# dspcraft/dsc

Measured on AMD Instinct MI355X. Metric: batched 1-D rfft GSamples/s, higher is better.
Workload: dtype f32

## Files before the change

dsc_amd/csrc/fft_r2c_64k.hip:

```cpp
#include "kernels.h"

#include <hip/hip_runtime.h>

#include <cmath>
#include <cstdlib>
#include <utility>

namespace {

typedef float f2 __attribute__((ext_vector_type(2)));

struct cf { float x, y; };
__device__ __forceinline__ cf operator+(cf a, cf b) { return cf{a.x + b.x, a.y + b.y}; }
__device__ __forceinline__ cf operator-(cf a, cf b) { return cf{a.x - b.x, a.y - b.y}; }
__device__ __forceinline__ cf to_cf(f2 a) { return cf{a.x, a.y}; }
__device__ __forceinline__ f2 to_f2(cf a) { return f2{a.x, a.y}; }

constexpr int kM = 32768;
constexpr int kRowPitch = 34;
constexpr int kPlaneFloats = 1024 * kRowPitch;
constexpr int kLdsBytes = kPlaneFloats * 4 + 1024 * 8;
constexpr int kTabEntries = 1024;

constexpr int kAuxW1024 = 0, kAuxW32768 = 1024, kAuxW65536 = 2048, kAuxEntries = 3072;

__host__ __device__ constexpr int br5(int x) {
    return ((x & 1) << 4) | ((x & 2) << 2) | (x & 4) | ((x & 8) >> 2) | ((x & 16) >> 4);
}

__device__ constexpr float kCos64[17] = {
    1.0f, 0.99518472667219688624f, 0.98078528040323044913f, 0.95694033573220886494f,
    0.92387953251128675613f, 0.88192126434835502971f, 0.83146961230254523708f, 0.77301045336273696081f,
    0.70710678118654752440f, 0.63439328416364549822f, 0.55557023301960222474f, 0.47139673682599764856f,
    0.38268343236508977173f, 0.29028467725446236764f, 0.19509032201612826785f, 0.09801714032956060199f,
    0.0f};

__device__ constexpr float root64_re(int q) {
    q &= 63;
    return q <= 16 ? kCos64[q] : q <= 32 ? -kCos64[32 - q] : q <= 48 ? -kCos64[q - 32] : kCos64[64 - q];
}
__device__ constexpr float root64_im(int q) {
    q &= 63;
    return q <= 16 ? -kCos64[16 - q] : q <= 32 ? -kCos64[q - 16] : q <= 48 ? kCos64[48 - q] : kCos64[q - 48];
}

__device__ __forceinline__ cf cmul(cf a, cf w) {
    return cf{a.x * w.x - a.y * w.y, a.x * w.y + a.y * w.x};
}
__device__ __forceinline__ cf cmul_conj(cf a, cf w) {
    return cf{a.x * w.x + a.y * w.y, a.y * w.x - a.x * w.y};
}

template<bool INV, int M, int K>
__device__ __forceinline__ cf mul_root(cf d) {
    constexpr float c8 = 0.70710678118654752440f;
    if constexpr (K == 0) {
        return d;
    } else if constexpr (4 * K == M) {
        return INV ? cf{-d.y, d.x} : cf{d.y, -d.x};
    } else if constexpr (8 * K == M) {
        return INV ? cf{(d.x - d.y) * c8, (d.x + d.y) * c8} : cf{(d.x + d.y) * c8, (d.y - d.x) * c8};
    } else if constexpr (8 * K == 3 * M) {
        return INV ? cf{-(d.x + d.y) * c8, (d.x - d.y) * c8} : cf{(d.y - d.x) * c8, -(d.x + d.y) * c8};
    } else {
        constexpr float wr = root64_re(K * (64 / M));
        constexpr float wi = INV ? -root64_im(K * (64 / M)) : root64_im(K * (64 / M));
        return cf{d.x * wr - d.y * wi, d.x * wi + d.y * wr};
    }
}

#ifdef DSC_DFT32_DIF
template<bool INV, int M, int G, int... K>
__device__ __forceinline__ void dif_group(cf (&v)[32], std::integer_sequence<int, K...>) {
    (([&] {
         const cf u = v[G + K] + v[G + K + M / 2];
         const cf d = v[G + K] - v[G + K + M / 2];
         v[G + K] = u;
         v[G + K + M / 2] = mul_root<INV, M, K>(d);
     }()),
     ...);
}

template<bool INV, int M, int... G>
__device__ __forceinline__ void dif_stage(cf (&v)[32], std::integer_sequence<int, G...>) {
    (dif_group<INV, M, G * M>(v, std::make_integer_sequence<int, M / 2>{}), ...);
}

template<bool INV>
__device__ __forceinline__ void dft32(cf (&v)[32]) {
    dif_stage<INV, 32>(v, std::make_integer_sequence<int, 1>{});
    dif_stage<INV, 16>(v, std::make_integer_sequence<int, 2>{});
    dif_stage<INV, 8>(v, std::make_integer_sequence<int, 4>{});
    dif_stage<INV, 4>(v, std::make_integer_sequence<int, 8>{});
    dif_stage<INV, 2>(v, std::make_integer_sequence<int, 16>{});
}


#else
constexpr double kCos64d[17] = {
    1.0, 0.99518472667219688624, 0.98078528040323044913, 0.95694033573220886494,
    0.92387953251128675613, 0.88192126434835502971, 0.83146961230254523708, 0.77301045336273696081,
    0.70710678118654752440, 0.63439328416364549822, 0.55557023301960222474, 0.47139673682599764856,
    0.38268343236508977173, 0.29028467725446236764, 0.19509032201612826785, 0.09801714032956060199,
    0.0};

template<bool INV, int E>
__device__ __forceinline__ void dit_butterfly(cf &a, cf &b) {
    if constexpr (E == 0) {
        const cf u = a + b, d = a - b;
        a = u; b = d;
    } else if constexpr (E == 8) {
        const cf u = INV ? cf{a.x - b.y, a.y + b.x} : cf{a.x + b.y, a.y - b.x};
        const cf d = INV ? cf{a.x + b.y, a.y - b.x} : cf{a.x - b.y, a.y + b.x};
        a = u; b = d;
    } else {
        constexpr double c = E <= 8 ? kCos64d[2 * E] : -kCos64d[32 - 2 * E];
        constexpr double sn = (E <= 8 ? kCos64d[16 - 2 * E] : kCos64d[2 * E - 16]);
        constexpr double s = INV ? sn : -sn;
        if constexpr ((c < 0 ? -c : c) >= sn) {
            constexpr float t = (float) (s / c), cc = (float) c;
            float p, q;
            if constexpr (t == 1.0f) { p = b.x - b.y; q = b.y + b.x; }
            else if constexpr (t == -1.0f) { p = b.x + b.y; q = b.y - b.x; }
            else { p = __builtin_fmaf(-t, b.y, b.x); q = __builtin_fmaf(t, b.x, b.y); }
            const cf u = cf{__builtin_fmaf(cc, p, a.x), __builtin_fmaf(cc, q, a.y)};
            const cf d = cf{__builtin_fmaf(-cc, p, a.x), __builtin_fmaf(-cc, q, a.y)};
            a = u; b = d;
        } else {
            constexpr float r = (float) (c / s), ss = (float) s;
            const float pn = __builtin_fmaf(-r, b.x, b.y);
            const float q = __builtin_fmaf(r, b.y, b.x);
            const cf u = cf{__builtin_fmaf(-ss, pn, a.x), __builtin_fmaf(ss, q, a.y)};
            const cf d = cf{__builtin_fmaf(ss, pn, a.x), __builtin_fmaf(-ss, q, a.y)};
            a = u; b = d;
        }
    }
}

constexpr int brev_bits(int x, int bits) {
    int r = 0;
    for (int i = 0; i < bits; ++i) r |= ((x >> i) & 1) << (bits - 1 - i);
    return r;
}

template<bool INV, int S, int G, int... J>
__device__ __forceinline__ void dit_group(cf (&v)[32], std::integer_sequence<int, J...>) {
    constexpr int H = 32 >> S;
    constexpr int E = brev_bits(G, S - 1) * (16 >> (S - 1));
    (dit_butterfly<INV, E>(v[2 * H * G + J], v[2 * H * G + J + H]), ...);
}

template<bool INV, int S, int... G>
__device__ __forceinline__ void dit_stage(cf (&v)[32], std::integer_sequence<int, G...>) {
    (dit_group<INV, S, G>(v, std::make_integer_sequence<int, (32 >> S)>{}), ...);
}

template<bool INV>
__device__ __forceinline__ void dft32(cf (&v)[32]) {
    dit_stage<INV, 1>(v, std::make_integer_sequence<int, 1>{});
    dit_stage<INV, 2>(v, std::make_integer_sequence<int, 2>{});
    dit_stage<INV, 3>(v, std::make_integer_sequence<int, 4>{});
    dit_stage<INV, 4>(v, std::make_integer_sequence<int, 8>{});
    dit_stage<INV, 5>(v, std::make_integer_sequence<int, 16>{});
}
#endif

typedef unsigned int u2 __attribute__((ext_vector_type(2)));
typedef unsigned int u4 __attribute__((ext_vector_type(4)));
typedef float f4 __attribute__((ext_vector_type(4)));

template<int COMP>
__device__ __forceinline__ void plane_write(float *plane, int wbase, const cf (&v)[32]) {
    float *lo16 = plane + wbase;
    float *hi16 = lo16 + 16 * (32 * kRowPitch);
#pragma unroll
    for (int p = 0; p < 32; ++p) {
        const int slot = br5(p);
        const float val = COMP == 0 ? v[p].x : v[p].y;
        if (slot < 16) lo16[slot * (32 * kRowPitch)] = val;
        else           hi16[(slot - 16) * (32 * kRowPitch)] = val;
    }
}
template<int COMP>
__device__ __forceinline__ void plane_read(const float *plane, int row, cf (&v)[32]) {
    const f2 *r = (const f2 *) (plane + row * kRowPitch);
#pragma unroll
    for (int m = 0; m < 16; ++m) {
        const f2 t = r[m];
        if (COMP == 0) { v[2 * m].x = t.x; v[2 * m + 1].x = t.y; }
        else           { v[2 * m].y = t.x; v[2 * m + 1].y = t.y; }
    }
}

__device__ __forceinline__ void lds_barrier() {
    __builtin_amdgcn_fence(__ATOMIC_RELEASE, "workgroup", "local");
    __builtin_amdgcn_s_barrier();
    __builtin_amdgcn_fence(__ATOMIC_ACQUIRE, "workgroup", "local");
}

__device__ __forceinline__ float bperm(int byte_addr, float x) {
    return __int_as_float(__builtin_amdgcn_ds_bpermute(byte_addr, __float_as_int(x)));
}

__device__ __forceinline__ int column_of(int wave, int lane) {
    int kp = lane < 32 ? 32 * wave + lane : 1024 - 32 * wave - (63 - lane);
    return kp == 1024 ? 512 : kp;
}

#ifdef DSC_R2C64K_PROBE
#define PROBE_ARGS , int io_on
#define PROBE_NULL , 1
#define IO_ON io_on
#else
#define PROBE_ARGS
#define PROBE_NULL
#define IO_ON 1
#endif

__device__ __forceinline__ int thread_id(int wave_sgpr) {
    int zero;
    asm volatile("v_mov_b32 %0, 0" : "=v"(zero));
    const int lane = __builtin_amdgcn_mbcnt_hi(-1, __builtin_amdgcn_mbcnt_lo(-1, zero));
    return (wave_sgpr << 6) | lane;
}

#ifndef DSC_STREAM_AUX
#define DSC_STREAM_AUX 2
#endif
constexpr int kStream = DSC_STREAM_AUX;
__device__ __forceinline__ cf load_c(__amdgpu_buffer_rsrc_t r, int voff, int soff) {
    return to_cf(__builtin_bit_cast(f2, __builtin_amdgcn_raw_buffer_load_b64(r, voff, soff, kStream)));
}
#ifndef DSC_FILTER_EARLY_LOADS
#define DSC_FILTER_EARLY_LOADS 4
#endif
#ifndef DSC_IRFFT_PIN_PASS3
#define DSC_IRFFT_PIN_PASS3 1
#endif
#ifndef DSC_IRFFT_EARLY_PAIRS
#define DSC_IRFFT_EARLY_PAIRS 4
#endif
#ifndef DSC_IRFFT_LOAD_AUX
#define DSC_IRFFT_LOAD_AUX 0
#endif
__device__ __forceinline__ cf load_c_spec(__amdgpu_buffer_rsrc_t r, int voff, int soff) {
    return to_cf(__builtin_bit_cast(f2, __builtin_amdgcn_raw_buffer_load_b64(r, voff, soff, DSC_IRFFT_LOAD_AUX)));
}
__device__ __forceinline__ cf load_c_cached(__amdgpu_buffer_rsrc_t r, int voff, int soff) {
    return to_cf(__builtin_bit_cast(f2, __builtin_amdgcn_raw_buffer_load_b64(r, voff, soff, 0)));
}
template<int POLICY>
__device__ __forceinline__ void store_c(cf a, __amdgpu_buffer_rsrc_t r, int voff, int soff) {
    __builtin_amdgcn_raw_buffer_store_b64(__builtin_bit_cast(u2, to_f2(a)), r, voff, soff, POLICY);
}

__device__ __forceinline__ void exchange(float *plane, int wbase, int row, const cf (&src)[32], cf (&dst)[32]) {
    plane_write<0>(plane, wbase, src);
    lds_barrier();
    plane_read<0>(plane, row, dst);
    lds_barrier();
    plane_write<1>(plane, wbase, src);
    lds_barrier();
    plane_read<1>(plane, row, dst);
    lds_barrier();
}

struct no_hook { __device__ __forceinline__ void operator()() const {} };

template<bool INV, typename Hook = no_hook>
__device__ __forceinline__ void three_passes(cf (&v)[32], float *plane, const f2 *w1024, const f2 *aux, int wave_sgpr,
                                             bool mirrored_in, bool mirrored_out, Hook before_pass3 = Hook{}) {
    dft32<INV>(v);
    cf u[32];
    {
        const int t = thread_id(wave_sgpr);
        const int col = mirrored_in ? column_of(t >> 6, t & 63) : t;
        const int hi = col >> 5;
#pragma unroll
        for (int r1 = 1; r1 < 32; ++r1) {
            const cf w = to_cf(w1024[hi * r1]);
            v[br5(r1)] = INV ? cmul_conj(v[br5(r1)], w) : cmul(v[br5(r1)], w);
        }
        exchange(plane, (col & 31) * kRowPitch + hi, t, v, u);
    }
    dft32<INV>(u);
    {
        const int t = thread_id(wave_sgpr);
        const int hi = t >> 5, lo = t & 31;
        const cf tw2_base = to_cf(aux[kAuxW32768 + hi * lo]);
        u[0] = INV ? cmul_conj(u[0], tw2_base) : cmul(u[0], tw2_base);
#pragma unroll
        for (int r2 = 1; r2 < 32; ++r2) {
            const cf w = cmul(tw2_base, to_cf(w1024[lo * r2]));
            u[br5(r2)] = INV ? cmul_conj(u[br5(r2)], w) : cmul(u[br5(r2)], w);
        }
        const int col_out = mirrored_out ? column_of(t >> 6, t & 63) : t;
        exchange(plane, hi * kRowPitch + lo, col_out, u, v);
    }
    before_pass3();
    dft32<INV>(v);
}

__device__ __forceinline__ void real_pair(cf p, cf q, cf wq, float hs, cf &out_k, cf &out_mk) {
    const cf s = cf{p.x + q.x, p.y - q.y};
    const cf d = cf{p.x - q.x, p.y + q.y};
    const cf wd = cmul(d, wq);
    out_k = cf{hs * s.x + wd.x, hs * s.y + wd.y};
    out_mk = cf{hs * s.x - wd.x, wd.y - hs * s.y};
}

__device__ __forceinline__ int partner_byte_addr(int wave, int lane) {
    return ((wave == 0 && (lane == 63 || lane == 0)) ? lane : 63 - lane) * 4;
}

#ifndef DSC_R2C64K_HELPERS_ONLY
__global__ __launch_bounds__(1024) void rfft64k_kernel(const float *__restrict__ x, f2 *__restrict__ X, int batch,
                                                       const f2 *__restrict__ aux, int in_pitch, int in_len PROBE_ARGS) {
    extern __shared__ __attribute__((aligned(16))) float lds[];
    float *plane = lds;
    f2 *w1024 = (f2 *) (lds + kPlaneFloats);
    w1024[threadIdx.x] = aux[kAuxW1024 + threadIdx.x];
    __syncthreads();

    const int wave_sgpr = __builtin_amdgcn_readfirstlane(threadIdx.x >> 6);

    cf v[32];
    {
        const int row0 = blockIdx.x;
        const __amdgpu_buffer_rsrc_t r0 = __builtin_amdgcn_make_buffer_rsrc(
            (void *) (x + (size_t) row0 * in_pitch), 0, row0 < batch ? in_len * 4 * IO_ON : 0, 0x00020000);
        const int load_off = thread_id(wave_sgpr) * 8;
#pragma unroll
        for (int j1 = 0; j1 < 32; ++j1) v[j1] = load_c(r0, load_off, j1 * 8192);
    }

    for (int row = blockIdx.x; row < batch; row += gridDim.x) {
        const int next_row = row + gridDim.x;
        const __amdgpu_buffer_rsrc_t rnext = __builtin_amdgcn_make_buffer_rsrc(
            (void *) (x + (size_t) next_row * in_pitch), 0, next_row < batch ? in_len * 4 * IO_ON : 0, 0x00020000);
        const __amdgpu_buffer_rsrc_t rout =
            __builtin_amdgcn_make_buffer_rsrc((void *) (X + (size_t) row * (kM + 1)), 0, (kM + 1) * 8 * IO_ON, 0x00020000);

        three_passes<false>(v, plane, w1024, aux, wave_sgpr, false, true);

        const int t4 = thread_id(wave_sgpr);
        const int lane = t4 & 63, wave = t4 >> 6;
        const int kp = column_of(wave, lane);
        const int partner_addr = partner_byte_addr(wave, lane);
        cf xk[16], xm[16];
        const cf zmid = v[br5(16)];
        if (wave_sgpr == 0) {
#pragma unroll
            for (int r = 16; r < 31; ++r) v[br5(r)] = lane == 0 ? v[br5(r + 1)] : v[br5(r)];
            v[br5(31)] = lane == 0 ? v[br5(0)] : v[br5(31)];
        }
#pragma unroll
        for (int k3 = 0; k3 < 16; ++k3) {
            const int src = 31 - br5(k3);
            xm[k3].x = bperm(partner_addr, v[src].x);
            xm[k3].y = bperm(partner_addr, v[src].y);
        }
        {
            const cf wpost = to_cf(aux[kAuxW65536 + kp]);
            const cf post_base = cf{0.5f * wpost.y, -0.5f * wpost.x};
#pragma unroll
            for (int k3 = 0; k3 < 16; ++k3) {
                const cf c = cf{root64_re(k3), root64_im(k3)};
                const cf w = k3 == 0 ? post_base : cmul(post_base, c);
                real_pair(v[br5(k3)], xm[k3], w, 0.5f, xk[k3], xm[k3]);
            }
        }

        f2 *stage = (f2 *) plane;
        const int skew = (int) ((((size_t) (X + (size_t) row * (kM + 1))) >> 3) & 15);
#pragma unroll
        for (int k3 = 0; k3 < 16; ++k3) stage[kp + 1024 * k3] = to_f2(xk[k3]);
        const cf xk15 = xk[15];
        const int load_off = thread_id(wave_sgpr) * 8;
#pragma unroll
        for (int j1 = 0; j1 < 16; ++j1) v[j1] = load_c(rnext, load_off, j1 * 8192);
        lds_barrier();
#pragma unroll
        for (int m = 0; m < 8; ++m) {
            const int k = 2 * (t4 + 1024 * m) - skew;
            if (m > 0 || k >= 0) {
                const f2 lo2 = stage[k], hi2 = stage[k + 1];
                const f4 q = f4{lo2.x, lo2.y, hi2.x, hi2.y};
                __builtin_amdgcn_raw_buffer_store_b128(__builtin_bit_cast(u4, q), rout, k * 8, 0, kStream);
            } else if (m == 0 && k == -1) {
                __builtin_amdgcn_raw_buffer_store_b64(__builtin_bit_cast(u2, stage[0]), rout, 0, 0, kStream);
            }
            if (m & 1) __builtin_amdgcn_sched_barrier(0);
        }
        lds_barrier();
        constexpr int kStage2 = kM / 2 - 16;
#pragma unroll
        for (int k3 = 0; k3 < 16; ++k3) stage[(kM - kStage2) - kp - 1024 * k3] = to_f2(xm[k3]);
        if (kp >= 1009) stage[kp + 15 * 1024 - kStage2] = to_f2(xk15);
        if (t4 == 0) stage[kM / 2 - kStage2] = f2{zmid.x, -zmid.y};
#pragma unroll
        for (int j1 = 16; j1 < 32; ++j1) v[j1] = load_c(rnext, load_off, j1 * 8192);
        lds_barrier();
#pragma unroll
        for (int m = 0; m < 9; ++m) {
            if (m == 8 && wave != 0) break;
            const int k = kM / 2 + 2 * (t4 + 1024 * m) - skew;
            if (m < 8 || k + 1 <= kM) {
                const f2 lo2 = stage[k - kStage2], hi2 = stage[k + 1 - kStage2];
                const f4 q = f4{lo2.x, lo2.y, hi2.x, hi2.y};
                __builtin_amdgcn_raw_buffer_store_b128(__builtin_bit_cast(u4, q), rout, k * 8, 0, kStream);
            } else if (m == 8 && k == kM) {
                __builtin_amdgcn_raw_buffer_store_b64(__builtin_bit_cast(u2, stage[k - kStage2]), rout, k * 8, 0, kStream);
            }
            if (m & 1) __builtin_amdgcn_sched_barrier(0);
        }
        lds_barrier();
    }
}

#endif

__device__ __forceinline__ void inverse_prepass_direct(cf (&v)[32], cf y_mid, const f2 *aux, int wave_sgpr) {
    constexpr float kScale = 1.0f / (float) kM;
    const int t1 = thread_id(wave_sgpr);
    const int lane = t1 & 63, wave = t1 >> 6;
    const int c = column_of(wave, lane);
    const int partner_addr = partner_byte_addr(wave, lane);
    if (wave == 0 && lane == 0) { v[0].y = 0.f; v[16].y = 0.f; }
    const cf wpre = to_cf(aux[kAuxW65536 + c]);
    const cf wq_base = cf{0.5f * kScale * wpre.y, 0.5f * kScale * wpre.x};
#pragma unroll
    for (int half = 0; half < 2; ++half) {
        cf zm[8];
#pragma unroll
        for (int i = 0; i < 8; ++i) {
            const int a = half * 8 + i;
            const cf cj = cf{root64_re(a), -root64_im(a)};
            const cf wq = a == 0 ? wq_base : cmul(wq_base, cj);
            real_pair(v[a], v[16 + a], wq, 0.5f * kScale, v[a], zm[i]);
        }
#pragma unroll
        for (int i = 0; i < 8; ++i) {
            const int a = half * 8 + i;
            v[16 + a].x = bperm(partner_addr, zm[i].x);
            v[16 + a].y = bperm(partner_addr, zm[i].y);
        }
    }
    cf w[32];
#pragma unroll
    for (int r = 0; r < 16; ++r) { w[r] = v[r]; w[16 + r] = v[31 - r]; }
    if (wave == 0) {
#pragma unroll
        for (int r = 31; r > 16; --r) w[r] = lane == 0 ? w[r - 1] : w[r];
        w[16] = lane == 0 ? cf{kScale * y_mid.x, -kScale * y_mid.y} : w[16];
    }
#pragma unroll
    for (int r = 0; r < 32; ++r) v[r] = w[r];
}

template<typename IssueNext>
__device__ __forceinline__ void staged_time_store(cf (&v)[32], float *plane, __amdgpu_buffer_rsrc_t rout, int wave_sgpr,
                                                  IssueNext issue_next) {
    f2 *stage = (f2 *) plane;
    const int t4 = thread_id(wave_sgpr);
#pragma unroll
    for (int p = 0; p < 32; p += 2) stage[t4 + 1024 * br5(p)] = to_f2(v[p]);
    issue_next(true);
    lds_barrier();
#pragma unroll
    for (int m = 0; m < 8; ++m) {
        const int k = 2 * (t4 + 1024 * m);
        const f2 lo2 = stage[k], hi2 = stage[k + 1];
        const f4 q = f4{lo2.x, lo2.y, hi2.x, hi2.y};
        __builtin_amdgcn_raw_buffer_store_b128(__builtin_bit_cast(u4, q), rout, k * 8, 0, kStream);
        if (m & 1) __builtin_amdgcn_sched_barrier(0);
    }
    lds_barrier();
#pragma unroll
    for (int p = 1; p < 32; p += 2) stage[t4 + 1024 * (br5(p) - 16)] = to_f2(v[p]);
    issue_next(false);
    lds_barrier();
#pragma unroll
    for (int m = 0; m < 8; ++m) {
        const int k = 2 * (t4 + 1024 * m);
        const f2 lo2 = stage[k], hi2 = stage[k + 1];
        const f4 q = f4{lo2.x, lo2.y, hi2.x, hi2.y};
        __builtin_amdgcn_raw_buffer_store_b128(__builtin_bit_cast(u4, q), rout, (kM / 2 + k) * 8, 0, kStream);
        if (m & 1) __builtin_amdgcn_sched_barrier(0);
    }
    lds_barrier();
}

__device__ __forceinline__ void unzip_rows(cf (&v)[32]) {
    cf nxt[32];
#pragma unroll
    for (int a = 0; a < 16; ++a) { nxt[a] = v[2 * a]; nxt[16 + a] = v[2 * a + 1]; }
#pragma unroll
    for (int a = 0; a < 32; ++a) v[a] = nxt[a];
}

#ifndef DSC_R2C64K_HELPERS_ONLY
__global__ __launch_bounds__(1024) void irfft64k_kernel(const f2 *__restrict__ X, float *__restrict__ x, int batch,
                                                        const f2 *__restrict__ aux, int in_pitch, int in_len PROBE_ARGS) {
    extern __shared__ __attribute__((aligned(16))) float lds[];
    float *plane = lds;
    f2 *w1024 = (f2 *) (lds + kPlaneFloats);
    w1024[threadIdx.x] = aux[kAuxW1024 + threadIdx.x];
    __syncthreads();

    const int wave_sgpr = __builtin_amdgcn_readfirstlane(threadIdx.x >> 6);

    cf v[32];
    cf y_mid = cf{0.f, 0.f};
    {
        const int row0 = blockIdx.x;
        const __amdgpu_buffer_rsrc_t r0 = __builtin_amdgcn_make_buffer_rsrc(
            (void *) (X + (size_t) row0 * in_pitch), 0, row0 < batch ? in_len * 8 * IO_ON : 0, 0x00020000);
        const int t0 = thread_id(wave_sgpr);
        const int c = column_of(t0 >> 6, t0 & 63);
        const int pv = (kM - c - 15 * 1024) * 8;
#pragma unroll
        for (int a = 0; a < 16; ++a) {
            v[a] = load_c_spec(r0, c * 8, a * 8192);
            v[16 + a] = load_c_spec(r0, pv, (15 - a) * 8192);
        }
        if (c == 0) y_mid = load_c_spec(r0, (kM / 2) * 8, 0);
    }

    for (int row = blockIdx.x; row < batch; row += gridDim.x) {
        const int next_row = row + gridDim.x;
        const __amdgpu_buffer_rsrc_t rnext = __builtin_amdgcn_make_buffer_rsrc(
            (void *) (X + (size_t) next_row * in_pitch), 0, next_row < batch ? in_len * 8 * IO_ON : 0, 0x00020000);
        const __amdgpu_buffer_rsrc_t rout =
            __builtin_amdgcn_make_buffer_rsrc((void *) (x + (size_t) row * 65536), 0, 65536 * 4 * IO_ON, 0x00020000);

        inverse_prepass_direct(v, y_mid, aux, wave_sgpr);
        constexpr int kEarly = DSC_IRFFT_EARLY_PAIRS;
        cf early[kEarly > 0 ? 2 * kEarly : 1];
        three_passes<true>(v, plane, w1024, aux, wave_sgpr, true, false, [&]() {
            if constexpr (kEarly > 0) {
                const int t3 = thread_id(wave_sgpr);
                const int c3 = column_of(t3 >> 6, t3 & 63);
                const int pv3 = (kM - c3 - 15 * 1024) * 8;
#pragma unroll
                for (int a = 0; a < kEarly; ++a) {
                    early[2 * a] = load_c_spec(rnext, c3 * 8, a * 8192);
                    early[2 * a + 1] = load_c_spec(rnext, pv3, (15 - a) * 8192);
                }
            }
        });

#if DSC_IRFFT_PIN_PASS3
#pragma unroll
        for (int p = 0; p < 32; p += 8)
            asm volatile("" : "+v"(v[p].x), "+v"(v[p].y), "+v"(v[p + 1].x), "+v"(v[p + 1].y), "+v"(v[p + 2].x), "+v"(v[p + 2].y), "+v"(v[p + 3].x),
                         "+v"(v[p + 3].y), "+v"(v[p + 4].x), "+v"(v[p + 4].y), "+v"(v[p + 5].x), "+v"(v[p + 5].y), "+v"(v[p + 6].x), "+v"(v[p + 6].y),
                         "+v"(v[p + 7].x), "+v"(v[p + 7].y));
#endif
        const int t4 = thread_id(wave_sgpr);
        const int c = column_of(t4 >> 6, t4 & 63);
        const int pv = (kM - c - 15 * 1024) * 8;
        staged_time_store(v, plane, rout, wave_sgpr, [&](bool first_half) {
            if (first_half) {
                y_mid = cf{0.f, 0.f};
                if (c == 0) y_mid = load_c_spec(rnext, (kM / 2) * 8, 0);
#pragma unroll
                for (int i = 0; i < 8; ++i) {
                    v[2 * i] = load_c_spec(rnext, c * 8, (kEarly + i) * 8192);
                    v[16 + 2 * i] = load_c_spec(rnext, pv, (15 - kEarly - i) * 8192);
                }
            } else {
#pragma unroll
                for (int i = 0; i < 8 - kEarly; ++i) {
                    v[2 * i + 1] = load_c_spec(rnext, c * 8, (kEarly + 8 + i) * 8192);
                    v[17 + 2 * i] = load_c_spec(rnext, pv, (7 - kEarly - i) * 8192);
                }
            }
        });
        {
            cf nxt[32];
#pragma unroll
            for (int a = 0; a < 16; ++a) {
                if (a < kEarly)          { nxt[a] = early[2 * a];             nxt[16 + a] = early[2 * a + 1]; }
                else if (a < kEarly + 8) { nxt[a] = v[2 * (a - kEarly)];      nxt[16 + a] = v[16 + 2 * (a - kEarly)]; }
                else                     { nxt[a] = v[2 * (a - kEarly - 8) + 1]; nxt[16 + a] = v[17 + 2 * (a - kEarly - 8)]; }
            }
#pragma unroll
            for (int a = 0; a < 32; ++a) v[a] = nxt[a];
        }
    }
}

__global__ __launch_bounds__(1024) void filter64k_kernel(const float *__restrict__ x, const f2 *__restrict__ H,
                                                         float *__restrict__ y, int batch, const f2 *__restrict__ aux, int in_pitch,
                                                         int in_len) {
    extern __shared__ __attribute__((aligned(16))) float lds[];
    float *plane = lds;
    f2 *w1024 = (f2 *) (lds + kPlaneFloats);
    w1024[threadIdx.x] = aux[kAuxW1024 + threadIdx.x];
    __syncthreads();

    const int wave_sgpr = __builtin_amdgcn_readfirstlane(threadIdx.x >> 6);
    const __amdgpu_buffer_rsrc_t rh = __builtin_amdgcn_make_buffer_rsrc((void *) H, 0, (kM + 1) * 8, 0x00020000);
    constexpr float kScale = 1.0f / (float) kM;

    cf v[32];
    {
        const int row0 = blockIdx.x;
        const __amdgpu_buffer_rsrc_t r0 = __builtin_amdgcn_make_buffer_rsrc(
            (void *) (x + (size_t) row0 * in_pitch), 0, row0 < batch ? in_len * 4 : 0, 0x00020000);
        const int load_off = thread_id(wave_sgpr) * 8;
#pragma unroll
        for (int j1 = 0; j1 < 32; ++j1) v[j1] = load_c(r0, load_off, j1 * 8192);
    }
    for (int row = blockIdx.x; row < batch; row += gridDim.x) {
        const int next_row = row + gridDim.x;
        const __amdgpu_buffer_rsrc_t rnext = __builtin_amdgcn_make_buffer_rsrc(
            (void *) (x + (size_t) next_row * in_pitch), 0, next_row < batch ? in_len * 4 : 0, 0x00020000);
        const __amdgpu_buffer_rsrc_t rout =
            __builtin_amdgcn_make_buffer_rsrc((void *) (y + (size_t) row * 65536), 0, 65536 * 4, 0x00020000);
        three_passes<false>(v, plane, w1024, aux, wave_sgpr, false, true);

        {
            const int t1 = thread_id(wave_sgpr);
            const int lane = t1 & 63, wave = t1 >> 6;
            const int c = column_of(wave, lane);
            const int partner_addr = partner_byte_addr(wave, lane);
            const cf wc = to_cf(aux[kAuxW65536 + c]);
            const cf post_base = cf{0.5f * wc.y, -0.5f * wc.x};
            const cf pre_base = cf{0.5f * kScale * wc.y, 0.5f * kScale * wc.x};
            if (wave == 0) {
                const cf zmid = v[br5(16)];
                const cf hmid = load_c_cached(rh, (kM / 2) * 8, 0);
                const cf pmid = cmul(cf{zmid.x, -zmid.y}, hmid);
                v[br5(16)] = lane == 0 ? cf{kScale * pmid.x, -kScale * pmid.y} : v[br5(16)];
            }
            cf park = v[br5(16)];
            if (wave == 0) {
#pragma unroll
                for (int r = 16; r < 31; ++r) v[br5(r)] = lane == 0 ? v[br5(r + 1)] : v[br5(r)];
                v[br5(31)] = lane == 0 ? v[br5(0)] : v[br5(31)];
            }
#pragma unroll
            for (int part = 0; part < 8; ++part) {
                cf q[2], zm[2];
#pragma unroll
                for (int i = 0; i < 2; ++i) {
                    const int a = part * 2 + i;
                    q[i].x = bperm(partner_addr, v[br5(31 - a)].x);
                    q[i].y = bperm(partner_addr, v[br5(31 - a)].y);
                }
#pragma unroll
                for (int i = 0; i < 2; ++i) {
                    const int a = part * 2 + i;
                    const cf w64 = cf{root64_re(a), root64_im(a)};
                    cf xk, xm;
                    real_pair(v[br5(a)], q[i], a == 0 ? post_base : cmul(post_base, w64), 0.5f, xk, xm);
                    const cf hk = load_c_cached(rh, c * 8, a * 8192);
                    const cf hm = load_c_cached(rh, (kM - 15 * 1024 - c) * 8, (15 - a) * 8192);
                    cf pk = cmul(xk, hk), pm = cmul(xm, hm);
                    if (a == 0) {
                        pk.y = (c == 0) ? 0.f : pk.y;
                        pm.y = (c == 0) ? 0.f : pm.y;
                    }
                    const cf w64c = cf{root64_re(a), -root64_im(a)};
                    real_pair(pk, pm, a == 0 ? pre_base : cmul(pre_base, w64c), 0.5f * kScale, v[br5(a)], zm[i]);
                }
#pragma unroll
                for (int i = 0; i < 2; ++i) {
                    const int a = part * 2 + i;
                    v[br5(31 - a)].x = bperm(partner_addr, zm[i].x);
                    v[br5(31 - a)].y = bperm(partner_addr, zm[i].y);
                }
                __builtin_amdgcn_sched_barrier(0);
            }
            if (wave == 0) {
#pragma unroll
                for (int r = 31; r > 16; --r) v[br5(r)] = lane == 0 ? v[br5(r - 1)] : v[br5(r)];
                v[br5(16)] = lane == 0 ? park : v[br5(16)];
            }
        }
        cf z[32];
#pragma unroll
        for (int r = 0; r < 32; ++r) z[r] = v[br5(r)];
        constexpr int kEarlyX = DSC_FILTER_EARLY_LOADS;
        cf early[kEarlyX > 0 ? kEarlyX : 1];
        three_passes<true>(z, plane, w1024, aux, wave_sgpr, true, false, [&]() {
            if constexpr (kEarlyX > 0) {
                const int off = thread_id(wave_sgpr) * 8;
#pragma unroll
                for (int j1 = 0; j1 < kEarlyX; ++j1) early[j1] = load_c(rnext, off, j1 * 8192);
            }
        });
        {
            const int load_off = thread_id(wave_sgpr) * 8;
            staged_time_store(z, plane, rout, wave_sgpr, [&](bool first_half) {
                if (first_half) {
#pragma unroll
                    for (int i = 0; i < 16; ++i) z[2 * i] = load_c(rnext, load_off, (kEarlyX + i) * 8192);
                } else {
#pragma unroll
                    for (int i = 0; i < 16 - kEarlyX; ++i) z[2 * i + 1] = load_c(rnext, load_off, (kEarlyX + 16 + i) * 8192);
                }
            });
#pragma unroll
            for (int j1 = 0; j1 < 32; ++j1) v[j1] = j1 < kEarlyX ? early[j1] : j1 < kEarlyX + 16 ? z[2 * (j1 - kEarlyX)] : z[2 * (j1 - kEarlyX - 16) + 1];
        }
    }
}

#endif

}

#ifndef DSC_R2C64K_HELPERS_ONLY
size_t dsc_r2c64k_table_bytes() { return (size_t) kAuxEntries * sizeof(float) * 2; }

void dsc_r2c64k_build_tables(void *host_dst) {
    float *o = (float *) host_dst;
    auto put = [&](int at, long long k, long long n) {
        const long double a = -2.0L * 3.14159265358979323846264338327950288L * (long double) k / (long double) n;
        o[2 * at] = (float) cosl(a);
        o[2 * at + 1] = (float) sinl(a);
    };
    for (int m = 0; m < kTabEntries; ++m) {
        put(kAuxW1024 + m, m, 1024);
        put(kAuxW32768 + m, m, 32768);
        put(kAuxW65536 + m, m, 65536);
    }
    o[2 * (kAuxW1024 + 256)] = 0.f;  o[2 * (kAuxW1024 + 256) + 1] = -1.f;
    o[2 * (kAuxW1024 + 512)] = -1.f; o[2 * (kAuxW1024 + 512) + 1] = 0.f;
    o[2 * (kAuxW1024 + 768)] = 0.f;  o[2 * (kAuxW1024 + 768) + 1] = 1.f;
}

void dsc_launch_rfft64k(const float *x, void *X, int batch, int in_pitch, int in_len, const void *aux, int n_cu, hipStream_t stream) {
    if (batch <= 0) return;
    static unsigned long long attr_devices = 0;
    if (dsc_first_use_on_device(attr_devices)) {
        DSC_KERNEL_CHECK(hipFuncSetAttribute((const void *) rfft64k_kernel, hipFuncAttributeMaxDynamicSharedMemorySize, kLdsBytes));
    }
    const int grid = batch < n_cu ? batch : n_cu;
    DSC_LAUNCH(rfft64k_kernel, dim3(grid), dim3(1024), kLdsBytes, stream, x, (f2 *) X, batch, (const f2 *) aux, in_pitch, in_len PROBE_NULL);
}

void dsc_launch_irfft64k(const void *X, float *x, int batch, int in_pitch, int in_len, const void *aux, int n_cu, hipStream_t stream) {
    if (batch <= 0) return;
    static unsigned long long attr_devices = 0;
    if (dsc_first_use_on_device(attr_devices)) {
        DSC_KERNEL_CHECK(hipFuncSetAttribute((const void *) irfft64k_kernel, hipFuncAttributeMaxDynamicSharedMemorySize, kLdsBytes));
    }
    const int grid = batch < n_cu ? batch : n_cu;
    DSC_LAUNCH(irfft64k_kernel, dim3(grid), dim3(1024), kLdsBytes, stream, (const f2 *) X, x, batch, (const f2 *) aux, in_pitch, in_len PROBE_NULL);
}
void dsc_launch_filter64k(const float *s, const void *H, float *y, int batch, int in_pitch, int in_len, const void *aux, int n_cu,
                          hipStream_t stream) {
    if (batch <= 0) return;
    static unsigned long long attr_devices = 0;
    if (dsc_first_use_on_device(attr_devices)) {
        DSC_KERNEL_CHECK(hipFuncSetAttribute((const void *) filter64k_kernel, hipFuncAttributeMaxDynamicSharedMemorySize, kLdsBytes));
    }
    const int grid = batch < n_cu ? batch : n_cu;
    DSC_LAUNCH(filter64k_kernel, dim3(grid), dim3(1024), kLdsBytes, stream, s, (const f2 *) H, y, batch, (const f2 *) aux, in_pitch, in_len);
}
#endif
```

dsc_amd/csrc/fft_c2c_32k.hip:

```cpp
#define DSC_R2C64K_HELPERS_ONLY 1
#include "fft_r2c_64k.hip"

namespace {

template<bool INV, bool CAST>
__global__ __launch_bounds__(1024) void c2c32k_kernel(const f2 *__restrict__ z, f2 *__restrict__ Z, int batch, const f2 *__restrict__ aux,
                                                      int in_pitch, int in_len) {
    constexpr int EB = CAST ? 4 : 8;
    auto sample = [](__amdgpu_buffer_rsrc_t r, int voff, int soff) {
        if constexpr (CAST) return cf{__builtin_bit_cast(float, __builtin_amdgcn_raw_buffer_load_b32(r, voff, soff, kStream)), 0.0f};
        else return load_c(r, voff, soff);
    };
    extern __shared__ __attribute__((aligned(16))) float lds[];
    float *plane = lds;
    f2 *w1024 = (f2 *) (lds + kPlaneFloats);
    w1024[threadIdx.x] = aux[kAuxW1024 + threadIdx.x];
    __syncthreads();
    const int wave_sgpr = __builtin_amdgcn_readfirstlane(threadIdx.x >> 6);
    constexpr float kScale = 1.0f / (float) kM;

    cf v[32];
    {
        const int row0 = blockIdx.x;
        const __amdgpu_buffer_rsrc_t r0 = __builtin_amdgcn_make_buffer_rsrc(
            (void *) ((const char *) z + (size_t) row0 * in_pitch * EB), 0, row0 < batch ? in_len * EB : 0, 0x00020000);
        const int load_off = thread_id(wave_sgpr) * EB;
#pragma unroll
        for (int a = 0; a < 32; ++a) v[a] = sample(r0, load_off, a * 1024 * EB);
    }
    for (int row = blockIdx.x; row < batch; row += gridDim.x) {
        const int next_row = row + gridDim.x;
        const __amdgpu_buffer_rsrc_t rnext = __builtin_amdgcn_make_buffer_rsrc(
            (void *) ((const char *) z + (size_t) next_row * in_pitch * EB), 0, next_row < batch ? in_len * EB : 0, 0x00020000);
        const __amdgpu_buffer_rsrc_t rout = __builtin_amdgcn_make_buffer_rsrc((void *) (Z + (size_t) row * kM), 0, kM * 8, 0x00020000);
        three_passes<INV>(v, plane, w1024, aux, wave_sgpr, false, false);
        if (INV) {
#pragma unroll
            for (int p = 0; p < 32; ++p) v[p] = cf{v[p].x * kScale, v[p].y * kScale};
        }
        const int load_off = thread_id(wave_sgpr) * EB;
        staged_time_store(v, plane, rout, wave_sgpr, [&](bool first_half) {
            if (first_half) {
#pragma unroll
                for (int a = 0; a < 16; ++a) v[2 * a] = sample(rnext, load_off, a * 1024 * EB);
            } else {
#pragma unroll
                for (int a = 16; a < 32; ++a) v[2 * (a - 16) + 1] = sample(rnext, load_off, a * 1024 * EB);
            }
        });
        unzip_rows(v);
    }
}

}

void dsc_launch_fft32k_c32(const void *z, void *Z, int batch, int in_pitch, int in_len, bool inverse, bool cast, const void *aux, int n_cu,
                           hipStream_t stream) {
    if (batch <= 0) return;
    static unsigned long long attr_devices = 0;
    if (dsc_first_use_on_device(attr_devices)) {
        DSC_KERNEL_CHECK(hipFuncSetAttribute((const void *) c2c32k_kernel<false, false>, hipFuncAttributeMaxDynamicSharedMemorySize, kLdsBytes));
        DSC_KERNEL_CHECK(hipFuncSetAttribute((const void *) c2c32k_kernel<true, false>, hipFuncAttributeMaxDynamicSharedMemorySize, kLdsBytes));
        DSC_KERNEL_CHECK(hipFuncSetAttribute((const void *) c2c32k_kernel<false, true>, hipFuncAttributeMaxDynamicSharedMemorySize, kLdsBytes));
        DSC_KERNEL_CHECK(hipFuncSetAttribute((const void *) c2c32k_kernel<true, true>, hipFuncAttributeMaxDynamicSharedMemorySize, kLdsBytes));
    }
    const int grid = batch < n_cu ? batch : n_cu;
#define C2C32K(INV, CAST) DSC_LAUNCH((c2c32k_kernel<INV, CAST>), dim3(grid), dim3(1024), kLdsBytes, stream, (const f2 *) z, (f2 *) Z, batch, (const f2 *) aux, in_pitch, in_len)
    if (inverse) { if (cast) C2C32K(true, true); else C2C32K(true, false); }
    else         { if (cast) C2C32K(false, true); else C2C32K(false, false); }
#undef C2C32K
}
```

Measured before the change: 639.3.

## Relayout twiddle table and LDS staging for constant-offset reads and aligned stores

The W1024 table is rebuilt as a 32x32 product table indexed by (a,b), so each twiddle fetch becomes a base address plus an immediate offset, with no per-element multiply. Plane reads are forced into sixteen back-to-back ds_read_b64 instructions in inline asm, and plane writes are split into two loops over the even and odd output slots. The output staging buffer is pre-shifted by the skew so each store reads a single aligned f4 from LDS instead of two f2 loads. The inline asm with a full lgkmcnt wait and memory clobber limits how the compiler can schedule around it, and the changed table layout has to stay consistent with any other users of w1024 (e.g. the inverse path).

```diff
diff --git a/dsc_amd/csrc/fft_r2c_64k.hip b/dsc_amd/csrc/fft_r2c_64k.hip
--- a/dsc_amd/csrc/fft_r2c_64k.hip
+++ b/dsc_amd/csrc/fft_r2c_64k.hip
@@ -172,23 +172,45 @@
 template<int COMP>
 __device__ __forceinline__ void plane_write(float *plane, int wbase, const cf (&v)[32]) {
     float *lo16 = plane + wbase;
-    float *hi16 = lo16 + 16 * (32 * kRowPitch);
-#pragma unroll
-    for (int p = 0; p < 32; ++p) {
-        const int slot = br5(p);
-        const float val = COMP == 0 ? v[p].x : v[p].y;
-        if (slot < 16) lo16[slot * (32 * kRowPitch)] = val;
-        else           hi16[(slot - 16) * (32 * kRowPitch)] = val;
-    }
+    int wbase_hi = wbase + 16 * (32 * kRowPitch);
+    asm volatile("" : "+v"(wbase_hi));
+    float *hi16 = plane + wbase_hi;
+#pragma unroll
+    for (int p = 0; p < 32; p += 2) lo16[br5(p) * (32 * kRowPitch)] = COMP == 0 ? v[p].x : v[p].y;
+#pragma unroll
+    for (int p = 1; p < 32; p += 2) hi16[(br5(p) - 16) * (32 * kRowPitch)] = COMP == 0 ? v[p].x : v[p].y;
 }
 template<int COMP>
 __device__ __forceinline__ void plane_read(const float *plane, int row, cf (&v)[32]) {
-    const f2 *r = (const f2 *) (plane + row * kRowPitch);
+    typedef __attribute__((address_space(3))) const float lds_cfloat;
+    const unsigned addr = (unsigned) (size_t) (lds_cfloat *) (plane + row * kRowPitch);
+    f2 t[16];
+    asm volatile(
+        "ds_read_b64 %0, %16\n\t"
+        "ds_read_b64 %1, %16 offset:8\n\t"
+        "ds_read_b64 %2, %16 offset:16\n\t"
+        "ds_read_b64 %3, %16 offset:24\n\t"
+        "ds_read_b64 %4, %16 offset:32\n\t"
+        "ds_read_b64 %5, %16 offset:40\n\t"
+        "ds_read_b64 %6, %16 offset:48\n\t"
+        "ds_read_b64 %7, %16 offset:56\n\t"
+        "ds_read_b64 %8, %16 offset:64\n\t"
+        "ds_read_b64 %9, %16 offset:72\n\t"
+        "ds_read_b64 %10, %16 offset:80\n\t"
+        "ds_read_b64 %11, %16 offset:88\n\t"
+        "ds_read_b64 %12, %16 offset:96\n\t"
+        "ds_read_b64 %13, %16 offset:104\n\t"
+        "ds_read_b64 %14, %16 offset:112\n\t"
+        "ds_read_b64 %15, %16 offset:120\n\t"
+        "s_waitcnt lgkmcnt(0)"
+        : "=&v"(t[0]), "=&v"(t[1]), "=&v"(t[2]), "=&v"(t[3]), "=&v"(t[4]), "=&v"(t[5]), "=&v"(t[6]), "=&v"(t[7]),
+          "=&v"(t[8]), "=&v"(t[9]), "=&v"(t[10]), "=&v"(t[11]), "=&v"(t[12]), "=&v"(t[13]), "=&v"(t[14]), "=&v"(t[15])
+        : "v"(addr)
+        : "memory");
 #pragma unroll
     for (int m = 0; m < 16; ++m) {
-        const f2 t = r[m];
-        if (COMP == 0) { v[2 * m].x = t.x; v[2 * m + 1].x = t.y; }
-        else           { v[2 * m].y = t.x; v[2 * m + 1].y = t.y; }
+        if (COMP == 0) { v[2 * m].x = t[m].x; v[2 * m + 1].x = t[m].y; }
+        else           { v[2 * m].y = t[m].x; v[2 * m + 1].y = t[m].y; }
     }
 }
 
@@ -252,6 +274,16 @@
 template<int POLICY>
 __device__ __forceinline__ void store_c(cf a, __amdgpu_buffer_rsrc_t r, int voff, int soff) {
     __builtin_amdgcn_raw_buffer_store_b64(__builtin_bit_cast(u2, to_f2(a)), r, voff, soff, POLICY);
+}
+
+typedef __attribute__((address_space(3))) const f2 lds_cf2;
+__device__ __forceinline__ unsigned twiddle_base(const f2 *table, int b) {
+    return (unsigned) (size_t) (lds_cf2 *) (table + b);
+}
+__device__ __forceinline__ cf twiddle(unsigned base, int a) {
+    unsigned addr;
+    asm("v_add_u32 %0, %2, %1" : "=v"(addr) : "v"(base), "i"(a * 256));
+    return to_cf(*(lds_cf2 *) (size_t) addr);
 }
 
 __device__ __forceinline__ void exchange(float *plane, int wbase, int row, const cf (&src)[32], cf (&dst)[32]) {
@@ -276,9 +308,10 @@
         const int t = thread_id(wave_sgpr);
         const int col = mirrored_in ? column_of(t >> 6, t & 63) : t;
         const int hi = col >> 5;
+        const unsigned tw_base = twiddle_base(w1024, hi);
 #pragma unroll
         for (int r1 = 1; r1 < 32; ++r1) {
-            const cf w = to_cf(w1024[hi * r1]);
+            const cf w = twiddle(tw_base, r1);
             v[br5(r1)] = INV ? cmul_conj(v[br5(r1)], w) : cmul(v[br5(r1)], w);
         }
         exchange(plane, (col & 31) * kRowPitch + hi, t, v, u);
@@ -289,9 +322,10 @@
         const int hi = t >> 5, lo = t & 31;
         const cf tw2_base = to_cf(aux[kAuxW32768 + hi * lo]);
         u[0] = INV ? cmul_conj(u[0], tw2_base) : cmul(u[0], tw2_base);
+        const unsigned tw_base = twiddle_base(w1024, lo);
 #pragma unroll
         for (int r2 = 1; r2 < 32; ++r2) {
-            const cf w = cmul(tw2_base, to_cf(w1024[lo * r2]));
+            const cf w = cmul(tw2_base, twiddle(tw_base, r2));
             u[br5(r2)] = INV ? cmul_conj(u[br5(r2)], w) : cmul(u[br5(r2)], w);
         }
         const int col_out = mirrored_out ? column_of(t >> 6, t & 63) : t;
@@ -373,8 +407,9 @@
 
         f2 *stage = (f2 *) plane;
         const int skew = (int) ((((size_t) (X + (size_t) row * (kM + 1))) >> 3) & 15);
-#pragma unroll
-        for (int k3 = 0; k3 < 16; ++k3) stage[kp + 1024 * k3] = to_f2(xk[k3]);
+        const f4 *stage4 = (const f4 *) plane;
+#pragma unroll
+        for (int k3 = 0; k3 < 16; ++k3) stage[kp + skew + 1024 * k3] = to_f2(xk[k3]);
         const cf xk15 = xk[15];
         const int load_off = thread_id(wave_sgpr) * 8;
 #pragma unroll
@@ -383,21 +418,19 @@
 #pragma unroll
         for (int m = 0; m < 8; ++m) {
             const int k = 2 * (t4 + 1024 * m) - skew;
+            const f4 q = stage4[t4 + 1024 * m];
             if (m > 0 || k >= 0) {
-                const f2 lo2 = stage[k], hi2 = stage[k + 1];
-                const f4 q = f4{lo2.x, lo2.y, hi2.x, hi2.y};
                 __builtin_amdgcn_raw_buffer_store_b128(__builtin_bit_cast(u4, q), rout, k * 8, 0, kStream);
             } else if (m == 0 && k == -1) {
-                __builtin_amdgcn_raw_buffer_store_b64(__builtin_bit_cast(u2, stage[0]), rout, 0, 0, kStream);
+                __builtin_amdgcn_raw_buffer_store_b64(__builtin_bit_cast(u2, f2{q.z, q.w}), rout, 0, 0, kStream);
             }
             if (m & 1) __builtin_amdgcn_sched_barrier(0);
         }
         lds_barrier();
-        constexpr int kStage2 = kM / 2 - 16;
-#pragma unroll
-        for (int k3 = 0; k3 < 16; ++k3) stage[(kM - kStage2) - kp - 1024 * k3] = to_f2(xm[k3]);
-        if (kp >= 1009) stage[kp + 15 * 1024 - kStage2] = to_f2(xk15);
-        if (t4 == 0) stage[kM / 2 - kStage2] = f2{zmid.x, -zmid.y};
+#pragma unroll
+        for (int k3 = 0; k3 < 16; ++k3) stage[kM / 2 + skew - kp - 1024 * k3] = to_f2(xm[k3]);
+        if (kp + skew >= 1024) stage[kp + skew - 1024] = to_f2(xk15);
+        if (t4 == 0) stage[skew] = f2{zmid.x, -zmid.y};
 #pragma unroll
         for (int j1 = 16; j1 < 32; ++j1) v[j1] = load_c(rnext, load_off, j1 * 8192);
         lds_barrier();
@@ -405,12 +438,11 @@
         for (int m = 0; m < 9; ++m) {
             if (m == 8 && wave != 0) break;
             const int k = kM / 2 + 2 * (t4 + 1024 * m) - skew;
+            const f4 q = stage4[t4 + 1024 * m];
             if (m < 8 || k + 1 <= kM) {
-                const f2 lo2 = stage[k - kStage2], hi2 = stage[k + 1 - kStage2];
-                const f4 q = f4{lo2.x, lo2.y, hi2.x, hi2.y};
                 __builtin_amdgcn_raw_buffer_store_b128(__builtin_bit_cast(u4, q), rout, k * 8, 0, kStream);
             } else if (m == 8 && k == kM) {
-                __builtin_amdgcn_raw_buffer_store_b64(__builtin_bit_cast(u2, stage[k - kStage2]), rout, k * 8, 0, kStream);
+                __builtin_amdgcn_raw_buffer_store_b64(__builtin_bit_cast(u2, f2{q.x, q.y}), rout, k * 8, 0, kStream);
             }
             if (m & 1) __builtin_amdgcn_sched_barrier(0);
         }
@@ -724,13 +756,11 @@
         o[2 * at + 1] = (float) sinl(a);
     };
     for (int m = 0; m < kTabEntries; ++m) {
-        put(kAuxW1024 + m, m, 1024);
+        put(kAuxW1024 + m, (m >> 5) * (m & 31), 1024);
         put(kAuxW32768 + m, m, 32768);
         put(kAuxW65536 + m, m, 65536);
     }
-    o[2 * (kAuxW1024 + 256)] = 0.f;  o[2 * (kAuxW1024 + 256) + 1] = -1.f;
-    o[2 * (kAuxW1024 + 512)] = -1.f; o[2 * (kAuxW1024 + 512) + 1] = 0.f;
-    o[2 * (kAuxW1024 + 768)] = 0.f;  o[2 * (kAuxW1024 + 768) + 1] = 1.f;
+    o[2 * (kAuxW1024 + 16 * 32 + 16)] = 0.f;  o[2 * (kAuxW1024 + 16 * 32 + 16) + 1] = -1.f;
 }
 
 void dsc_launch_rfft64k(const float *x, void *X, int batch, int in_pitch, int in_len, const void *aux, int n_cu, hipStream_t stream) {
```

New measurement: 655.5, median of 4. +2.5%, better.

## Transpose twiddle table layout and split LDS plane accesses for cheaper addressing

Applied to the files above, without the earlier changes.

The LDS twiddle table now holds precomputed products, T[hi*32+r] = W1024[hi*r], so each per-thread twiddle lookup becomes a constant-stride offset from a per-thread base instead of a variable multiply index. plane_write is split into even and odd loops with an opaque hi-half base, and 24-bit multiplies are used for the LDS address math. LDS reads in plane_read and the staging stores go through a volatile 64-bit load helper to force split b64 reads. The aim is fewer VALU address computations and better ds instruction offsets. The volatile reads may limit how the compiler schedules or merges LDS loads.

```diff
diff --git a/dsc_amd/csrc/fft_c2c_32k.hip b/dsc_amd/csrc/fft_c2c_32k.hip
--- a/dsc_amd/csrc/fft_c2c_32k.hip
+++ b/dsc_amd/csrc/fft_c2c_32k.hip
@@ -13,9 +13,8 @@
     };
     extern __shared__ __attribute__((aligned(16))) float lds[];
     float *plane = lds;
-    f2 *w1024 = (f2 *) (lds + kPlaneFloats);
-    w1024[threadIdx.x] = aux[kAuxW1024 + threadIdx.x];
-    __syncthreads();
+    f2 *T = (f2 *) (lds + kPlaneFloats);
+    fill_twiddle_table(T, aux);
     const int wave_sgpr = __builtin_amdgcn_readfirstlane(threadIdx.x >> 6);
     constexpr float kScale = 1.0f / (float) kM;
 
@@ -33,7 +32,7 @@
         const __amdgpu_buffer_rsrc_t rnext = __builtin_amdgcn_make_buffer_rsrc(
             (void *) ((const char *) z + (size_t) next_row * in_pitch * EB), 0, next_row < batch ? in_len * EB : 0, 0x00020000);
         const __amdgpu_buffer_rsrc_t rout = __builtin_amdgcn_make_buffer_rsrc((void *) (Z + (size_t) row * kM), 0, kM * 8, 0x00020000);
-        three_passes<INV>(v, plane, w1024, aux, wave_sgpr, false, false);
+        three_passes<INV>(v, plane, T, aux, wave_sgpr, false, false);
         if (INV) {
 #pragma unroll
             for (int p = 0; p < 32; ++p) v[p] = cf{v[p].x * kScale, v[p].y * kScale};
diff --git a/dsc_amd/csrc/fft_r2c_64k.hip b/dsc_amd/csrc/fft_r2c_64k.hip
--- a/dsc_amd/csrc/fft_r2c_64k.hip
+++ b/dsc_amd/csrc/fft_r2c_64k.hip
@@ -171,22 +171,33 @@
 
 template<int COMP>
 __device__ __forceinline__ void plane_write(float *plane, int wbase, const cf (&v)[32]) {
+    int wbase_hi = wbase + 16 * (32 * kRowPitch);
+    asm("" : "+v"(wbase_hi));
     float *lo16 = plane + wbase;
-    float *hi16 = lo16 + 16 * (32 * kRowPitch);
-#pragma unroll
-    for (int p = 0; p < 32; ++p) {
-        const int slot = br5(p);
-        const float val = COMP == 0 ? v[p].x : v[p].y;
-        if (slot < 16) lo16[slot * (32 * kRowPitch)] = val;
-        else           hi16[(slot - 16) * (32 * kRowPitch)] = val;
-    }
-}
+    float *hi16 = plane + wbase_hi;
+#pragma unroll
+    for (int p = 0; p < 32; p += 2) lo16[br5(p) * (32 * kRowPitch)] = COMP == 0 ? v[p].x : v[p].y;
+#pragma unroll
+    for (int p = 1; p < 32; p += 2) hi16[(br5(p) - 16) * (32 * kRowPitch)] = COMP == 0 ? v[p].x : v[p].y;
+}
+
+#ifndef DSC_LDS_SPLIT_READS
+#define DSC_LDS_SPLIT_READS 1
+#endif
+__device__ __forceinline__ f2 lds_read_b64(const f2 *p) {
+#if DSC_LDS_SPLIT_READS
+    return *(const volatile __attribute__((address_space(3))) f2 *) p;
+#else
+    return *p;
+#endif
+}
+
 template<int COMP>
 __device__ __forceinline__ void plane_read(const float *plane, int row, cf (&v)[32]) {
-    const f2 *r = (const f2 *) (plane + row * kRowPitch);
+    const f2 *r = (const f2 *) (plane + __mul24(row, kRowPitch));
 #pragma unroll
     for (int m = 0; m < 16; ++m) {
-        const f2 t = r[m];
+        const f2 t = lds_read_b64(r + m);
         if (COMP == 0) { v[2 * m].x = t.x; v[2 * m + 1].x = t.y; }
         else           { v[2 * m].y = t.x; v[2 * m + 1].y = t.y; }
     }
@@ -252,6 +263,12 @@
 template<int POLICY>
 __device__ __forceinline__ void store_c(cf a, __amdgpu_buffer_rsrc_t r, int voff, int soff) {
     __builtin_amdgcn_raw_buffer_store_b64(__builtin_bit_cast(u2, to_f2(a)), r, voff, soff, POLICY);
+}
+
+__device__ __forceinline__ void fill_twiddle_table(f2 *T, const f2 *aux) {
+    const int t = threadIdx.x;
+    T[t] = aux[kAuxW1024 + (t >> 5) * (t & 31)];
+    __syncthreads();
 }
 
 __device__ __forceinline__ void exchange(float *plane, int wbase, int row, const cf (&src)[32], cf (&dst)[32]) {
@@ -268,7 +285,7 @@
 struct no_hook { __device__ __forceinline__ void operator()() const {} };
 
 template<bool INV, typename Hook = no_hook>
-__device__ __forceinline__ void three_passes(cf (&v)[32], float *plane, const f2 *w1024, const f2 *aux, int wave_sgpr,
+__device__ __forceinline__ void three_passes(cf (&v)[32], float *plane, const f2 *T, const f2 *aux, int wave_sgpr,
                                              bool mirrored_in, bool mirrored_out, Hook before_pass3 = Hook{}) {
     dft32<INV>(v);
     cf u[32];
@@ -276,26 +293,28 @@
         const int t = thread_id(wave_sgpr);
         const int col = mirrored_in ? column_of(t >> 6, t & 63) : t;
         const int hi = col >> 5;
+        const f2 *th = T + hi;
 #pragma unroll
         for (int r1 = 1; r1 < 32; ++r1) {
-            const cf w = to_cf(w1024[hi * r1]);
+            const cf w = to_cf(th[32 * r1]);
             v[br5(r1)] = INV ? cmul_conj(v[br5(r1)], w) : cmul(v[br5(r1)], w);
         }
-        exchange(plane, (col & 31) * kRowPitch + hi, t, v, u);
+        exchange(plane, __mul24(col & 31, kRowPitch) + hi, t, v, u);
     }
     dft32<INV>(u);
     {
         const int t = thread_id(wave_sgpr);
         const int hi = t >> 5, lo = t & 31;
-        const cf tw2_base = to_cf(aux[kAuxW32768 + hi * lo]);
+        const cf tw2_base = to_cf(aux[kAuxW32768 + __mul24(hi, lo)]);
         u[0] = INV ? cmul_conj(u[0], tw2_base) : cmul(u[0], tw2_base);
+        const f2 *tl = T + lo;
 #pragma unroll
         for (int r2 = 1; r2 < 32; ++r2) {
-            const cf w = cmul(tw2_base, to_cf(w1024[lo * r2]));
+            const cf w = cmul(tw2_base, to_cf(tl[32 * r2]));
             u[br5(r2)] = INV ? cmul_conj(u[br5(r2)], w) : cmul(u[br5(r2)], w);
         }
         const int col_out = mirrored_out ? column_of(t >> 6, t & 63) : t;
-        exchange(plane, hi * kRowPitch + lo, col_out, u, v);
+        exchange(plane, __mul24(hi, kRowPitch) + lo, col_out, u, v);
     }
     before_pass3();
     dft32<INV>(v);
@@ -318,9 +337,8 @@
                                                        const f2 *__restrict__ aux, int in_pitch, int in_len PROBE_ARGS) {
     extern __shared__ __attribute__((aligned(16))) float lds[];
     float *plane = lds;
-    f2 *w1024 = (f2 *) (lds + kPlaneFloats);
-    w1024[threadIdx.x] = aux[kAuxW1024 + threadIdx.x];
-    __syncthreads();
+    f2 *T = (f2 *) (lds + kPlaneFloats);
+    fill_twiddle_table(T, aux);
 
     const int wave_sgpr = __builtin_amdgcn_readfirstlane(threadIdx.x >> 6);
 
@@ -341,7 +359,7 @@
         const __amdgpu_buffer_rsrc_t rout =
             __builtin_amdgcn_make_buffer_rsrc((void *) (X + (size_t) row * (kM + 1)), 0, (kM + 1) * 8 * IO_ON, 0x00020000);
 
-        three_passes<false>(v, plane, w1024, aux, wave_sgpr, false, true);
+        three_passes<false>(v, plane, T, aux, wave_sgpr, false, true);
 
         const int t4 = thread_id(wave_sgpr);
         const int lane = t4 & 63, wave = t4 >> 6;
@@ -384,7 +402,7 @@
         for (int m = 0; m < 8; ++m) {
             const int k = 2 * (t4 + 1024 * m) - skew;
             if (m > 0 || k >= 0) {
-                const f2 lo2 = stage[k], hi2 = stage[k + 1];
+                const f2 lo2 = lds_read_b64(stage + k), hi2 = lds_read_b64(stage + k + 1);
                 const f4 q = f4{lo2.x, lo2.y, hi2.x, hi2.y};
                 __builtin_amdgcn_raw_buffer_store_b128(__builtin_bit_cast(u4, q), rout, k * 8, 0, kStream);
             } else if (m == 0 && k == -1) {
@@ -406,7 +424,7 @@
             if (m == 8 && wave != 0) break;
             const int k = kM / 2 + 2 * (t4 + 1024 * m) - skew;
             if (m < 8 || k + 1 <= kM) {
-                const f2 lo2 = stage[k - kStage2], hi2 = stage[k + 1 - kStage2];
+                const f2 lo2 = lds_read_b64(stage + k - kStage2), hi2 = lds_read_b64(stage + k + 1 - kStage2);
                 const f4 q = f4{lo2.x, lo2.y, hi2.x, hi2.y};
                 __builtin_amdgcn_raw_buffer_store_b128(__builtin_bit_cast(u4, q), rout, k * 8, 0, kStream);
             } else if (m == 8 && k == kM) {
@@ -470,7 +488,7 @@
 #pragma unroll
     for (int m = 0; m < 8; ++m) {
         const int k = 2 * (t4 + 1024 * m);
-        const f2 lo2 = stage[k], hi2 = stage[k + 1];
+        const f2 lo2 = lds_read_b64(stage + k), hi2 = lds_read_b64(stage + k + 1);
         const f4 q = f4{lo2.x, lo2.y, hi2.x, hi2.y};
         __builtin_amdgcn_raw_buffer_store_b128(__builtin_bit_cast(u4, q), rout, k * 8, 0, kStream);
         if (m & 1) __builtin_amdgcn_sched_barrier(0);
@@ -483,7 +501,7 @@
 #pragma unroll
     for (int m = 0; m < 8; ++m) {
         const int k = 2 * (t4 + 1024 * m);
-        const f2 lo2 = stage[k], hi2 = stage[k + 1];
+        const f2 lo2 = lds_read_b64(stage + k), hi2 = lds_read_b64(stage + k + 1);
         const f4 q = f4{lo2.x, lo2.y, hi2.x, hi2.y};
         __builtin_amdgcn_raw_buffer_store_b128(__builtin_bit_cast(u4, q), rout, (kM / 2 + k) * 8, 0, kStream);
         if (m & 1) __builtin_amdgcn_sched_barrier(0);
@@ -504,9 +522,8 @@
                                                         const f2 *__restrict__ aux, int in_pitch, int in_len PROBE_ARGS) {
     extern __shared__ __attribute__((aligned(16))) float lds[];
     float *plane = lds;
-    f2 *w1024 = (f2 *) (lds + kPlaneFloats);
-    w1024[threadIdx.x] = aux[kAuxW1024 + threadIdx.x];
-    __syncthreads();
+    f2 *T = (f2 *) (lds + kPlaneFloats);
+    fill_twiddle_table(T, aux);
 
     const int wave_sgpr = __builtin_amdgcn_readfirstlane(threadIdx.x >> 6);
 
@@ -537,7 +554,7 @@
         inverse_prepass_direct(v, y_mid, aux, wave_sgpr);
         constexpr int kEarly = DSC_IRFFT_EARLY_PAIRS;
         cf early[kEarly > 0 ? 2 * kEarly : 1];
-        three_passes<true>(v, plane, w1024, aux, wave_sgpr, true, false, [&]() {
+        three_passes<true>(v, plane, T, aux, wave_sgpr, true, false, [&]() {
             if constexpr (kEarly > 0) {
                 const int t3 = thread_id(wave_sgpr);
                 const int c3 = column_of(t3 >> 6, t3 & 63);
@@ -596,9 +613,8 @@
                                                          int in_len) {
     extern __shared__ __attribute__((aligned(16))) float lds[];
     float *plane = lds;
-    f2 *w1024 = (f2 *) (lds + kPlaneFloats);
-    w1024[threadIdx.x] = aux[kAuxW1024 + threadIdx.x];
-    __syncthreads();
+    f2 *T = (f2 *) (lds + kPlaneFloats);
+    fill_twiddle_table(T, aux);
 
     const int wave_sgpr = __builtin_amdgcn_readfirstlane(threadIdx.x >> 6);
     const __amdgpu_buffer_rsrc_t rh = __builtin_amdgcn_make_buffer_rsrc((void *) H, 0, (kM + 1) * 8, 0x00020000);
@@ -619,7 +635,7 @@
             (void *) (x + (size_t) next_row * in_pitch), 0, next_row < batch ? in_len * 4 : 0, 0x00020000);
         const __amdgpu_buffer_rsrc_t rout =
             __builtin_amdgcn_make_buffer_rsrc((void *) (y + (size_t) row * 65536), 0, 65536 * 4, 0x00020000);
-        three_passes<false>(v, plane, w1024, aux, wave_sgpr, false, true);
+        three_passes<false>(v, plane, T, aux, wave_sgpr, false, true);
 
         {
             const int t1 = thread_id(wave_sgpr);
@@ -685,7 +701,7 @@
         for (int r = 0; r < 32; ++r) z[r] = v[br5(r)];
         constexpr int kEarlyX = DSC_FILTER_EARLY_LOADS;
         cf early[kEarlyX > 0 ? kEarlyX : 1];
-        three_passes<true>(z, plane, w1024, aux, wave_sgpr, true, false, [&]() {
+        three_passes<true>(z, plane, T, aux, wave_sgpr, true, false, [&]() {
             if constexpr (kEarlyX > 0) {
                 const int off = thread_id(wave_sgpr) * 8;
 #pragma unroll
```

New measurement: 639.1 before, 659.5 after (median of 6 runs). 1.03x the previous value.
